# QuantumLiquids/PEPS

Hardware: AMD Instinct MI355X
Metric: configuration-amplitudes/sec (higher is better)
Workload: dtype f32

## Files before the change

### include/pepsgpu.h

```cpp
#ifndef PEPSGPU_H
#define PEPSGPU_H

#include <stddef.h>
#include <stdint.h>

#ifdef __cplusplus
extern "C" {
#endif

typedef struct pepsgpu_ctx pepsgpu_ctx;

enum {
  PEPSGPU_OK = 0,
  PEPSGPU_EINVAL = 1,
  PEPSGPU_EHIP = 2,
  PEPSGPU_ESTATE = 3,
  PEPSGPU_ERANGE = 4,
  PEPSGPU_EEMPTY = 5,
  PEPSGPU_ENOCONV = 6
};
enum { PEPSGPU_F32 = 0, PEPSGPU_F64 = 1, PEPSGPU_C128 = 3 };
enum { PEPSGPU_LEFT = 0, PEPSGPU_DOWN = 1, PEPSGPU_RIGHT = 2, PEPSGPU_UP = 3 };
enum { PEPSGPU_HORIZONTAL = 0, PEPSGPU_VERTICAL = 1 };
enum { PEPSGPU_SVD_COMPRESS = 0, PEPSGPU_VARIATION2SITE = 1, PEPSGPU_VARIATION1SITE = 2 };
// ... 203 lines not shown
int pepsgpu_comm_destroy(pepsgpu_ctx *ctx);
int pepsgpu_allreduce(pepsgpu_ctx *ctx, void *buf, long n, int dtype, int op, int on_device);
int pepsgpu_grad_allreduce(pepsgpu_ctx *ctx);
int pepsgpu_bcast_state(pepsgpu_ctx *ctx, int root);
int pepsgpu_grad_device_ptr(pepsgpu_ctx *ctx, void **so_dev, void **seo_dev, long *n_elems);

int pepsgpu_diag_tgemm(int dtype_in, int dtype_out, const int *desc_ints, int n_ints, const void *A, size_t a_elems,
                       const void *B, size_t b_elems, void *C, size_t c_elems, int nbatch, long wA, long wB, long wC);
int pepsgpu_diag_tgemm_desc(int types, const int *desc_ints, int n_ints, const long *desc_longs, int n_longs,
                            const double *desc_dbls, int n_dbls, const int32_t *pool, long pool_n, const float *scale_in,
                            const void *A, size_t a_elems, long a_offset, const void *B, size_t b_elems, long b_offset,
                            void *C, size_t c_elems, float *scale_out, double *norm_log, int32_t *norm_flag,
                            int32_t *route_out, unsigned long long *flops_out);
int pepsgpu_diag_tgemm_route(int types, const int *desc_ints, int n_ints, const long *desc_longs, int n_longs,
                             const double *desc_dbls, int n_dbls, long a_offset, long b_offset, int32_t *route_out);
int pepsgpu_diag_tgemm_chain3(const int *dims8, const int *site_strides4, long slot, int nslots, const int32_t *sel, int sel_inc,
                              const int32_t *live4, const int32_t *skip, int nbatch, const int *offs3, const float *mps1,
                              const float *bten, const float *site, const float *mps2, float *out, int32_t *flags_out,
                              int32_t *launched_out, int32_t *variant_out);
int pepsgpu_diag_dot4(int dtype, const void *a, const void *b, const int *dims4, int nbatch, const double *lsum, const int32_t *flag,
                      double *out);
int pepsgpu_diag_chol(int dtype_out, const double *G, int n, int nbatch, void *R_out);
int pepsgpu_diag_gram_cols(int dtype, const void *P, int K, int n, int nbatch, const int32_t *klive, double *G_out);
int pepsgpu_diag_gram_rows(const float *M, int n, int K, int nbatch, const int32_t *nrows, double *G_out);
int pepsgpu_diag_mgemm_dense(const float *R, const float *Tt, int m, int la, int a_dim, int u_dim, int k2_dim, int tt_u_inner, int nbatch,
                             const int32_t *m_live, const int32_t *a_live, const int32_t *k2_live, float *M_out);
int pepsgpu_diag_cg_stats(double *out16);
int pepsgpu_diag_lds_gram_chol(int which, const float *X, int n, int K, int nbatch, const int32_t *nlive, float *R_out, int32_t *mlive_out);
int pepsgpu_diag_chol_pivot(const float *X, int n, int K, int nbatch, const int32_t *nlive, int kcap, float *R_out, int32_t *mlive_out);
int pepsgpu_diag_rows_qr(const float *X, int k, int len, int nbatch, const int32_t *klive, float *V_out, int32_t *klive_out);
int pepsgpu_diag_suwa_todo(const double *weights, int n, int init, const uint32_t *words, int steps, int32_t *out_chain);
int pepsgpu_diag_tgemm_chain(const int *dims7, const int32_t *live3_per_entry, int nbatch, const float *R, const float *A,
                             const float *W, float *P_out, int32_t *flags_out);
int pepsgpu_diag_gram_chol(int dtype, const void *P, int K, int n, int nbatch, void *R_out, int32_t *mlive_out);
int pepsgpu_diag_gram_chol_wave(const float *P, int K, int n, int nbatch, const int32_t *klive, int inner,
                                const int32_t *inner_live, int max_pass, int form, float *R_out, int32_t *mlive_out);
int pepsgpu_diag_chol_adaptive(int dtype_out, const double *G, int n, int nbatch, void *R_out, int32_t *mlive_out);
int pepsgpu_diag_jacobi(int dtype, void *M, int m, int len, int nbatch, int k, void *Vt_out, void *S_out,
                        int force_global, int *sweeps_out);
int pepsgpu_diag_chol_solve_rows(int is_complex, const void *S, void *X, int nbatch, int r_max, int len, const int32_t *rows, int r,
                                 const int32_t *run_flag);
int pepsgpu_diag_gather_rows(int is_complex, const void *M, int nbatch, int m, int len, const int32_t *piv, int slots,
                             const int32_t *rows, const int32_t *run_flag, void *Q);
int pepsgpu_diag_sign_table(int is_complex, int rows, int cols, void *out);
int pepsgpu_diag_truncate_site(pepsgpu_ctx *ctx, const void *M, int nbatch, int m, int u, int k2, const int32_t *rows, int route,
                               void *V_out, int32_t *klive_out, int32_t *route_flag_out);
int pepsgpu_diag_trunc_rows(const float *M, int m, int len, int nbatch, const int32_t *rows, int k, int span, float *Vt_out,
                            int32_t *klive_out, int32_t *sweeps_out);
const char *pepsgpu_version(void);

#ifdef __cplusplus
}
#endif
#endif
```

### peps_amd/capi.py

```python
import ctypes as C
import os

import numpy as np

_HERE = os.path.dirname(os.path.abspath(__file__))
LIB_PATH = os.environ.get("PEPSGPU_LIB") or os.path.join(_HERE, "lib", "libpepsgpu.so")

F32, F64 = 0, 1
C128 = 3
LEFT, DOWN, RIGHT, UP = 0, 1, 2, 3
HORIZONTAL, VERTICAL = 0, 1
LEFTUP_TO_RIGHTDOWN, LEFTDOWN_TO_RIGHTUP = 0, 1
SVD_COMPRESS, VARIATION2SITE, VARIATION1SITE = 0, 1, 2

_ERR = {1: ValueError, 2: RuntimeError, 3: RuntimeError, 4: IndexError, 5: RuntimeError}

SYMBOLS = [
    "pepsgpu_ctx_create", "pepsgpu_set_truncate_params", "pepsgpu_ctx_destroy", "pepsgpu_last_error", "pepsgpu_state_upload",
    "pepsgpu_walkers_set_configs", "pepsgpu_walkers_get_configs", "pepsgpu_n_walkers",
    "pepsgpu_grow_bmps_step", "pepsgpu_grow_full_bmps", "pepsgpu_grow_bmps_for_row", "pepsgpu_grow_bmps_for_col",
    "pepsgpu_shift_bmps_window", "pepsgpu_delete_inner_bmps", "pepsgpu_bmps_park", "pepsgpu_bmps_unpark", "pepsgpu_generate_bmps_approach",
    "pepsgpu_sweep_slice_exchange", "pepsgpu_sweep_slice_exchange_tab", "pepsgpu_sweep_slice_fullspace", "pepsgpu_sweep_slice_tnn3", "pepsgpu_diag_tnn3_table", "pepsgpu_nn_exchange_slice", "pepsgpu_nn_exchange_slice_tab", "pepsgpu_onsite_slice", "pepsgpu_nnn_exchange_slice", "pepsgpu_diag_nnn_slice_calls", "pepsgpu_nnn_hop_slice_fermion", "pepsgpu_diag_nnn_hop_slice_calls", "pepsgpu_diag_fermion_hop_cand", "pepsgpu_nn_pair_slice_fermion", "pepsgpu_diag_pair_slice_calls", "pepsgpu_diag_pair_cand", "pepsgpu_nn_hop_slice_fermion", "pepsgpu_diag_hop_slice_calls", "pepsgpu_sweep_slice_sector", "pepsgpu_diag_sector_slice_calls", "pepsgpu_diag_sector_cand", "pepsgpu_link_exchange_slice", "pepsgpu_diag_link_slice_calls", "pepsgpu_diag_link_cand", "pepsgpu_walker_create", "pepsgpu_walker_clone", "pepsgpu_walker_destroy", "pepsgpu_walker_info", "pepsgpu_walker_set_mpo", "pepsgpu_walker_set_mpo_excited", "pepsgpu_walker_trace_slice", "pepsgpu_diag_walker_slice_calls", "pepsgpu_walker_set_mpo_excited_pair", "pepsgpu_walker_pair_trace_slice", "pepsgpu_diag_walker_pair_slice_calls", "pepsgpu_diag_walker_pair_cand", "pepsgpu_walker_evolve",
    "pepsgpu_walker_evolve_step", "pepsgpu_walker_contract_row", "pepsgpu_walker_init_bten", "pepsgpu_walker_grow_bten_step",
    "pepsgpu_walker_shift_bten_window", "pepsgpu_walker_trace_with_bten", "pepsgpu_walker_clear_bten", "pepsgpu_walker_get_bmps_tensor",
    "pepsgpu_bmps_stack_size", "pepsgpu_get_bmps_tensor", "pepsgpu_init_bten", "pepsgpu_grow_full_bten",
    "pepsgpu_grow_bten_step", "pepsgpu_shift_bten_window", "pepsgpu_truncate_bten", "pepsgpu_bten_stack_size",
    "pepsgpu_trace", "pepsgpu_replace_nn_trace", "pepsgpu_replace_one_trace", "pepsgpu_trace_scaling", "pepsgpu_punch_hole",
    "pepsgpu_init_bten2", "pepsgpu_grow_full_bten2", "pepsgpu_grow_bten2_step", "pepsgpu_shift_bten2_window",
    "pepsgpu_bten2_stack_size", "pepsgpu_replace_nnn_trace", "pepsgpu_replace_tnn_trace",
    "pepsgpu_bten2_select_set", "pepsgpu_cfg_override_slice", "pepsgpu_replace_plaquette_trace",
    "pepsgpu_replace_sqrt5_trace",
    "pepsgpu_grad_reset", "pepsgpu_grad_accumulate", "pepsgpu_grad_accumulate_states", "pepsgpu_grad_read", "pepsgpu_grad_device_ptr", "pepsgpu_grad_allreduce", "pepsgpu_bcast_state",
    "pepsgpu_comm_unique_id", "pepsgpu_comm_init", "pepsgpu_comm_size", "pepsgpu_comm_rank", "pepsgpu_comm_destroy",
    "pepsgpu_allreduce",
    "pepsgpu_sr_begin", "pepsgpu_sr_append", "pepsgpu_sr_count", "pepsgpu_sr_sum", "pepsgpu_sr_matvec", "pepsgpu_sr_matvec_c128",
    "pepsgpu_sr_cg_solve", "pepsgpu_sr_gram", "pepsgpu_sr_weighted_sum", "pepsgpu_sr_copy_samples",
    "pepsgpu_opt_begin", "pepsgpu_opt_end", "pepsgpu_opt_gradient_from_accumulators", "pepsgpu_opt_set_gradient",
    "pepsgpu_opt_get_gradient", "pepsgpu_opt_clip", "pepsgpu_opt_natural_gradient", "pepsgpu_opt_step", "pepsgpu_opt_scale_state",
    "pepsgpu_opt_read_state", "pepsgpu_fermion_decoration_set", "pepsgpu_minsr_direction", "pepsgpu_diag_eigh",
    "pepsgpu_vmc_snapshot_save", "pepsgpu_vmc_snapshot_read", "pepsgpu_vmc_snapshot_clear",
    "pepsgpu_guard_base_save", "pepsgpu_guard_base_restore", "pepsgpu_guard_base_clear", "pepsgpu_guard_preview",
    "pepsgpu_lbfgs_begin", "pepsgpu_lbfgs_end", "pepsgpu_lbfgs_reset", "pepsgpu_lbfgs_update", "pepsgpu_lbfgs_direction",
    "pepsgpu_lbfgs_trial", "pepsgpu_lbfgs_slope", "pepsgpu_lbfgs_commit", "pepsgpu_lbfgs_get_direction", "pepsgpu_lbfgs_get_pair",
    "pepsgpu_lbfgs_counters",
    "pepsgpu_update_local", "pepsgpu_erase_envs_after_update", "pepsgpu_evaluate_amplitude",
    "pepsgpu_walker_flags", "pepsgpu_sync", "pepsgpu_stats", "pepsgpu_profile_enable", "pepsgpu_profile_read",
    "pepsgpu_diag_tgemm", "pepsgpu_diag_tgemm_desc", "pepsgpu_diag_tgemm_route", "pepsgpu_diag_tgemm_chain", "pepsgpu_diag_tgemm_chain3", "pepsgpu_diag_chol", "pepsgpu_diag_chol_adaptive", "pepsgpu_diag_chol_pivot", "pepsgpu_diag_rows_qr", "pepsgpu_diag_suwa_todo", "pepsgpu_diag_dot4", "pepsgpu_diag_gram_chol", "pepsgpu_diag_gram_chol_wave", "pepsgpu_diag_gram_cols", "pepsgpu_diag_gram_rows", "pepsgpu_diag_mgemm_dense", "pepsgpu_diag_jacobi", "pepsgpu_diag_trunc_rows", "pepsgpu_version",
    "pepsgpu_diag_chol_solve_rows", "pepsgpu_diag_gather_rows", "pepsgpu_diag_sign_table", "pepsgpu_diag_truncate_site",
]


def load_library(path=LIB_PATH):
    if not os.path.exists(path):
        raise ImportError("libpepsgpu.so not built (%s): run `python -c 'import __graft_entry__ as g; g.build()'`" % path)
    lib = C.CDLL(path)
    vp, ip, dp = C.c_void_p, C.POINTER(C.c_int32), C.POINTER(C.c_double)
    lib.pepsgpu_ctx_create.argtypes = [C.POINTER(vp)] + [C.c_int] * 8 + [C.c_double, C.c_int, C.c_int]
    lib.pepsgpu_set_truncate_params.argtypes = [vp, C.c_int, C.c_int, C.c_double, C.c_int, C.c_double, C.c_int]
    lib.pepsgpu_ctx_destroy.argtypes = [vp]
    lib.pepsgpu_ctx_destroy.restype = None
    lib.pepsgpu_last_error.argtypes = [vp]
    lib.pepsgpu_last_error.restype = C.c_char_p
    lib.pepsgpu_version.restype = C.c_char_p
    lib.pepsgpu_state_upload.argtypes = [vp, vp, C.c_int]
    lib.pepsgpu_walkers_set_configs.argtypes = [vp, C.c_int, ip]
    lib.pepsgpu_walkers_get_configs.argtypes = [vp, ip]
    lib.pepsgpu_n_walkers.argtypes = [vp]
    for name in ("grow_bmps_step", "grow_full_bmps", "grow_bmps_for_row", "grow_bmps_for_col", "shift_bmps_window",
                 "delete_inner_bmps", "generate_bmps_approach", "bmps_stack_size", "bten_stack_size",
                 "grow_bten_step", "shift_bten_window"):
        getattr(lib, "pepsgpu_" + name).argtypes = [vp, C.c_int]
    lib.pepsgpu_bmps_park.argtypes = [vp, C.c_int, C.c_int]
    lib.pepsgpu_bmps_unpark.argtypes = [vp, C.c_int]
    lib.pepsgpu_get_bmps_tensor.argtypes = [vp, C.c_int, C.c_int, C.c_int, ip, dp, dp]
    lib.pepsgpu_init_bten.argtypes = [vp, C.c_int, C.c_int]
    lib.pepsgpu_truncate_bten.argtypes = [vp, C.c_int, C.c_int]
    lib.pepsgpu_grow_full_bten.argtypes = [vp, C.c_int, C.c_int, C.c_int, C.c_int]
    lib.pepsgpu_trace.argtypes = [vp, C.c_int, C.c_int, C.c_int, dp]
    lib.pepsgpu_replace_nn_trace.argtypes = [vp, C.c_int, C.c_int, C.c_int, C.c_int, ip, dp]
    lib.pepsgpu_replace_one_trace.argtypes = [vp, C.c_int, C.c_int, C.c_int, C.c_int, ip, dp]
    lib.pepsgpu_punch_hole.argtypes = [vp, C.c_int, C.c_int, C.c_int, dp]
# ... 965 lines not shown
    if sel.size < (nb - 1) * sel_inc + 1 or (sv.size - int(o3[2])) < slot * (int(sel.max()) + 1):
        raise ValueError("diag_tgemm_chain3: selector or site store too small")
    flags = np.full(nb, 7, dtype=np.int32)
    launched = np.zeros(1, dtype=np.int32)
    variant = np.zeros(3, dtype=np.int32)
    vpp = lambda a: a.ctypes.data_as(C.c_void_p)
    rc = lib().pepsgpu_diag_tgemm_chain3(_ip(d8), _ip(st), slot, (sv.size - int(offs[2])) // slot, _ip(sel), sel_inc,
                                         None if lv is None else _ip(lv), None if sk is None else _ip(sk), nb, _ip(o3),
                                         vpp(m1), vpp(bt), vpp(sv), vpp(m2), vpp(out), _ip(flags), _ip(launched), _ip(variant))
    if rc != 0:
        raise RuntimeError("diag_tgemm_chain3 failed: %s" % lib().pepsgpu_last_error(None).decode())
    return out, flags, int(launched[0]), tuple(int(v) for v in variant)


def diag_tgemm_chain(R, A, W, live):
    R = np.ascontiguousarray(R, dtype=np.float32); A = np.ascontiguousarray(A, dtype=np.float32)
    W = np.ascontiguousarray(W, dtype=np.float32)
    nb, m, l, a = R.shape
    _, _, p, a2 = A.shape
    l2, u = W.shape[3], W.shape[4]
    dims = np.array([m, l, a, p, a2, l2, u], dtype=np.int32)
    lv = np.ascontiguousarray(live, dtype=np.int32)
    P = np.zeros((nb, m, u, l2, a2), dtype=np.float32)
    fl = np.zeros(nb, dtype=np.int32)
    f = lib().pepsgpu_diag_tgemm_chain
    f.argtypes = [C.POINTER(C.c_int32), C.POINTER(C.c_int32), C.c_int, C.c_void_p, C.c_void_p, C.c_void_p, C.c_void_p, C.POINTER(C.c_int32)]
    rc = f(_ip(dims), _ip(lv), nb, R.ctypes.data_as(C.c_void_p), A.ctypes.data_as(C.c_void_p), W.ctypes.data_as(C.c_void_p),
           P.ctypes.data_as(C.c_void_p), _ip(fl))
    if rc != 0:
        raise RuntimeError("diag_tgemm_chain failed: %s" % lib().pepsgpu_last_error(None).decode())
    return P, fl


def diag_chol(dtype_out, G):
    G = np.ascontiguousarray(G, dtype=np.float64)
    nb, n, _ = G.shape
    R = np.zeros((nb, n, n), dtype=np.float32 if dtype_out == F32 else np.float64)
    rc = lib().pepsgpu_diag_chol(dtype_out, _dp(G), n, nb, R.ctypes.data_as(C.c_void_p))
    if rc != 0:
        raise RuntimeError("diag_chol failed: %s" % lib().pepsgpu_last_error(None).decode())
    return R


def diag_chol_adaptive(dtype_out, G):
    G = np.ascontiguousarray(G, dtype=np.float64)
    nb, n, _ = G.shape
    R = np.zeros((nb, n, n), dtype=np.float32 if dtype_out == F32 else np.float64)
    ml = np.zeros(nb, dtype=np.int32)
    rc = lib().pepsgpu_diag_chol_adaptive(dtype_out, _dp(G), n, nb, R.ctypes.data_as(C.c_void_p), _ip(ml))
    if rc != 0:
        raise RuntimeError("diag_chol_adaptive failed: %s" % lib().pepsgpu_last_error(None).decode())
    return R, ml


def diag_gram_chol(dtype, P):
    t = np.float32 if dtype == F32 else np.float64
    P = np.ascontiguousarray(P, dtype=t)
    nb, K, n = P.shape
    R = np.zeros((nb, n, n), dtype=t)
    ml = np.zeros(nb, dtype=np.int32)
    rc = lib().pepsgpu_diag_gram_chol(dtype, P.ctypes.data_as(C.c_void_p), K, n, nb, R.ctypes.data_as(C.c_void_p), _ip(ml))
    if rc != 0:
        raise RuntimeError("diag_gram_chol failed: %s" % lib().pepsgpu_last_error(None).decode())
    return R, ml


# ... 462 lines not shown
```

### peps_amd/csrc/capi.hip

```cpp
#include <cstring>
#include "../../include/pepsgpu.h"
#include "engine_impl.h"
#include "engine_nnn.h"
#include "engine_sr.h"
#include "engine_opt.h"
#include "engine_lbfgs.h"
#include "engine_guard.h"
#include "engine_var.h"
#include "engine_cplx.h"
#include "engine_walker.h"
#include "engine_sweep.h"
#include "comm.h"

using namespace pepsgpu;

namespace pepsgpu {
bool tgemm_use_mfma() {
  static int v = -1;
  if (v < 0) {
    const char *e = getenv("PEPSGPU_NO_MFMA");
    v = (e && e[0] == '1') ? 0 : 1;
  }
  return v == 1;
}
// ... 837 lines not shown
    PG_CHECK_HIP(hipMalloc(&dl, 3 * (size_t)nbatch * sizeof(int)));
    PG_CHECK_HIP(hipMalloc(&dflag, nbatch * sizeof(int)));
    PG_CHECK_HIP(hipMemcpy(dR, R, nR * nbatch * sizeof(float), hipMemcpyHostToDevice));
    PG_CHECK_HIP(hipMemcpy(dA, A, nA * nbatch * sizeof(float), hipMemcpyHostToDevice));
    PG_CHECK_HIP(hipMemcpy(dW, W, nW * nbatch * sizeof(float), hipMemcpyHostToDevice));
    PG_CHECK_HIP(hipMemset(dP, 0, nP * nbatch * sizeof(float)));
    std::vector<int> hl(3 * (size_t)nbatch);
    for (int b = 0; b < nbatch; ++b)
      for (int q = 0; q < 3; ++q) hl[(size_t)q * nbatch + b] = live[3 * b + q];
    PG_CHECK_HIP(hipMemcpy(dl, hl.data(), hl.size() * sizeof(int), hipMemcpyHostToDevice));
    const int *ml = dl, *al = dl + nbatch, *a2l = dl + 2 * nbatch;
    TGemmDesc gx, gp;
    gx.I[1] = m; gx.I[2] = l; gx.sAi[1] = l * a; gx.sAi[2] = a; gx.sCi[1] = l * p * a2; gx.sCi[2] = p * a2;
    gx.K[2] = a; gx.sAk[2] = 1; gx.sBk[2] = p * a2;
    gx.J[1] = p; gx.J[2] = a2; gx.sBj[1] = a2; gx.sBj[2] = 1; gx.sCj[1] = a2; gx.sCj[2] = 1;
    gx.wA = (long)nR; gx.wB = (long)nA; gx.wC = 0; gx.nbatch = nbatch;
    gx.dI[1].p = ml; gx.dK[2].p = al; gx.dJ[2].p = a2l;
    gp.I[1] = l2; gp.I[2] = u; gp.sAi[1] = u; gp.sAi[2] = 1; gp.sCi[1] = a2; gp.sCi[2] = l2 * a2;
    gp.K[1] = l; gp.K[2] = p; gp.sAk[1] = p * l2 * u; gp.sAk[2] = l2 * u;
    gp.J[1] = m; gp.J[2] = a2; gp.sCj[1] = u * l2 * a2; gp.sCj[2] = 1;
    gp.wA = (long)nW; gp.wC = (long)nP; gp.nbatch = nbatch;
    gp.dJ[1].p = ml; gp.dJ[2].p = a2l;
    TGemmChainMap mp;
    mp.mapK[1] = 2; mp.mapK[2] = 4;
    mp.mapJ[1] = 1; mp.mapJ[2] = 5;
    const char *f64_s = getenv("PEPSGPU_DIAG_CHAIN_F64");
    const char *tri_s = getenv("PEPSGPU_DIAG_TRI");
    PG_REQUIRE(tgemm_chain_launch(0, gx, gp, mp, dR, dA, dW, dP, dflag, 1, tri_s && atoi(tri_s) ? 1 : 0, f64_s && atoi(f64_s) ? 1 : 0,
                                  tri_s && atoi(tri_s) ? 1 : 0), 1, "chain launch refused");
    PG_CHECK_HIP(hipDeviceSynchronize());
    PG_CHECK_HIP(hipMemcpy(P_out, dP, nP * nbatch * sizeof(float), hipMemcpyDeviceToHost));
    PG_CHECK_HIP(hipMemcpy(flags_out, dflag, nbatch * sizeof(int), hipMemcpyDeviceToHost));
    (void)hipFree(dR); (void)hipFree(dA); (void)hipFree(dW); (void)hipFree(dP); (void)hipFree(dl); (void)hipFree(dflag);
  });
}

template <typename T>
static void diag_chol_t(const double *G, int n, int nbatch, void *Rout) {
  double *dG;
  T *dR;
  size_t ne = (size_t)n * n * nbatch;
  PG_CHECK_HIP(hipMalloc(&dG, ne * sizeof(double)));
  PG_CHECK_HIP(hipMalloc(&dR, ne * sizeof(T)));
  PG_CHECK_HIP(hipMemcpy(dG, G, ne * sizeof(double), hipMemcpyHostToDevice));
  launch_chol_upper<T>(0, nbatch, dG, (long)n * n, n, dR, (long)n * n, (int *)nullptr);
  PG_CHECK_HIP(hipDeviceSynchronize());
  PG_CHECK_HIP(hipMemcpy(Rout, dR, ne * sizeof(T), hipMemcpyDeviceToHost));
  (void)hipFree(dG); (void)hipFree(dR);
}
template <typename T>
static void diag_chol_adaptive_t(const double *G, int n, int nbatch, void *Rout, int32_t *mlive) {
  double *dG;
  T *dR;
  int *dml;
  size_t ne = (size_t)n * n * nbatch;
  PG_REQUIRE(n <= 256 * CH_LR_Q, 1, "n too large for the low-rank Cholesky");
  PG_CHECK_HIP(hipMalloc(&dG, ne * sizeof(double)));
  PG_CHECK_HIP(hipMalloc(&dR, ne * sizeof(T)));
  PG_CHECK_HIP(hipMalloc(&dml, nbatch * sizeof(int)));
  PG_CHECK_HIP(hipMemcpy(dG, G, ne * sizeof(double), hipMemcpyHostToDevice));
  PG_CHECK_HIP(hipMemset(dR, 0, ne * sizeof(T)));
  const size_t lsm = chol_lowrank_smem_bytes(n), smem = chol_smem_bytes(n);
  allow_dynamic_lds(reinterpret_cast<const void *>(&chol_lowrank_kernel<T>), lsm);
  allow_dynamic_lds(reinterpret_cast<const void *>(&chol_upper_kernel<T>), smem);
  hipLaunchKernelGGL(chol_lowrank_kernel<T>, dim3(nbatch), dim3(256), lsm, 0, (const double *)dG, (long)n * n, n, dR,
                     (long)n * n, dml);
// ... 505 lines not shown
```

### peps_amd/csrc/tgemm.h

```cpp
#pragma once
#include "common.h"
#include "cplx.h"

namespace pepsgpu {

struct TgDyn {
  const int *p = nullptr;
  int mul = 1;
  int mask = 0;
  int div = 1;
};

struct TGemmDesc {
  int I[3] = {1, 1, 1}, J[3] = {1, 1, 1}, K[3] = {1, 1, 1};
  int sAi[3] = {0, 0, 0}, sAk[3] = {0, 0, 0};
  int sBk[3] = {0, 0, 0}, sBj[3] = {0, 0, 0};
  int sCi[3] = {0, 0, 0}, sCj[3] = {0, 0, 0};
  long wA = 0, wB = 0, wC = 0;
  const int *selA = nullptr, *selB = nullptr;
  int selA_inc = 0, selB_inc = 0;
  long selA_mul = 0, selB_mul = 0;
  int bdivA = 1, bdivB = 1, bdivC = 1;
  int seldivA = 1, seldivB = 1;
  const int *dynI = nullptr, *dynK = nullptr;
  int dynI_mul = 1, dynK_mul = 1;
  TgDyn dI[3], dJ[3], dK[3];
  int Imask[3] = {0x7fffffff, 0x7fffffff, 0x7fffffff}, Jmask[3] = {0x7fffffff, 0x7fffffff, 0x7fffffff};
  int nbatch = 1;
  int accumulate = 0;
  int upper_only = 0;
  int conjA = 0, conjB = 0;
  const int *batch_flag = nullptr;
  unsigned long long *flopc = nullptr;
// ... 1177 lines not shown
      if (s == jsub) d2.J[s] = cn;
      if (s == mp3.chunkI) { d3.I[s] = cn; d3.Imask[s] = 0x7fffffff; }
    }
    {
      int st = 1;
      for (int s = 2; s >= 0; --s) { lds1[3 + s] = st; st *= d1.J[s]; }
      for (int s = 2; s >= 0; --s) { lds1[s] = st; st *= d1.I[s]; }
      st = 1;
      for (int s = 2; s >= 0; --s) { lds2[3 + s] = st; st *= d2.J[s]; }
      for (int s = 2; s >= 0; --s) { lds2[s] = st; st *= d2.I[s]; }
    }
#pragma unroll
    for (int s = 0; s < 3; ++s) {
      d1.sCi[s] = lds1[s]; d1.sCj[s] = lds1[3 + s];
      d2.sBk[s] = mp.mapK[s] >= 0 ? lds1[mp.mapK[s]] : 0;
      d2.sBj[s] = mp.mapJ[s] >= 0 ? lds1[mp.mapJ[s]] : 0;
      d2.sCi[s] = lds2[s]; d2.sCj[s] = lds2[3 + s];
      d3.sAi[s] = mp3.mapI[s] >= 0 ? lds2[mp3.mapI[s]] : 0;
      d3.sAk[s] = mp3.mapK[s] >= 0 ? lds2[mp3.mapK[s]] : 0;
    }
    if (c0) __syncthreads();
    tg_direct_body<AVEC1, BVEC1>(d1, A1g + baseA1 + (long)c0 * sA1, B1g + baseB1, s_mid1, d1.Itot(), J1, K2s1, offCi_s, 0, 4, in_scale);
    __syncthreads();
    tg_direct_body<AVEC2, false>(d2, A2g + baseA2, s_mid1, s_mid2, I2, d2.Jtot(), K2s2, offCi_s, 0, 4);
    __syncthreads();
    tg_direct_body<false, false>(d3, s_mid2, B3g + baseB3, C3 + (long)c0 * sC3, d3.Itot(), J3, K2s3, offCi_s, 0, 4);
  }
  if (n1 < x_static) {
    const long lo = (long)n1 * sC3, hi = (long)x_static * sC3;
    for (long e = lo + threadIdx.x; e < hi; e += 256) C3[e] = 0.f;
  }
}

inline int tgemm_chain_launch(hipStream_t s, const TGemmDesc &d1_in, const TGemmDesc &d2_in, const TGemmChainMap &mp,
                              const float *A1, const float *B1, const float *A2, float *C2, int *flag, int allow_chunks = 0, int dense = 0,
                              int f64acc = 0, int tri = 0);

inline int tgemm_chain3_launch(hipStream_t s, const TGemmDesc &d1_in, const TGemmDesc &d2_in, const TGemmDesc &d3_in, const TGemmChainMap &mp,
                               const TGemmChain3Map &mp3, const float *A1, const float *B1, const float *A2, const float *B3, float *C3, int *flag,
                               const int *skip = nullptr);

struct BTenChainDescs {
  TGemmDesc g1, g2, g3;
  TGemmChainMap mp;
  TGemmChain3Map mp3;
};
inline BTenChainDescs bten_chain_descs(int x, int p1, int cdim, int b1, int b2, int s1, int s2, int y, int st_c, int st_b, int st_1,
                                       int st_2, long wA1, long wB1, long wB3, const int *sel, int sel_inc, long slot, int nb,
                                       const int *vx, const int *vc, const int *vb, const int *vy) {
  BTenChainDescs c;
  TGemmDesc &g1 = c.g1, &g2 = c.g2, &g3 = c.g3;
  g1.I[1] = x; g1.I[2] = p1; g1.sAi[1] = p1 * cdim; g1.sAi[2] = cdim; g1.sCi[1] = p1 * b1 * b2; g1.sCi[2] = b1 * b2;
  g1.K[2] = cdim; g1.sAk[2] = 1; g1.sBk[2] = b1 * b2;
  g1.J[1] = b1; g1.J[2] = b2; g1.sBj[1] = b2; g1.sBj[2] = 1; g1.sCj[1] = b2; g1.sCj[2] = 1;
  g1.wA = wA1; g1.wB = wB1; g1.wC = (long)x * p1 * b1 * b2; g1.nbatch = nb;
  g1.dI[1].p = vx; g1.dK[2].p = vc; g1.dJ[2].p = vb;
  g2.I[1] = s1; g2.I[2] = s2; g2.sAi[1] = st_1; g2.sAi[2] = st_2; g2.sCi[1] = s2; g2.sCi[2] = 1;
  g2.K[1] = p1; g2.K[2] = b1; g2.sAk[1] = st_c; g2.sAk[2] = st_b; g2.sBk[1] = b1 * b2; g2.sBk[2] = b2;
  g2.J[1] = x; g2.J[2] = b2; g2.sBj[1] = p1 * b1 * b2; g2.sBj[2] = 1; g2.sCj[1] = s1 * s2; g2.sCj[2] = x * s1 * s2;
  g2.wB = g1.wC; g2.wC = (long)b2 * x * s1 * s2; g2.nbatch = nb;
  g2.dJ[1].p = vx; g2.dJ[2].p = vb;
  g2.selA = sel; g2.selA_mul = slot; g2.selA_inc = sel_inc; g2.seldivA = 1; g2.wA = 0;
  c.mp.mapK[1] = 2; c.mp.mapK[2] = 4;
  c.mp.mapJ[1] = 1; c.mp.mapJ[2] = 5;
  g3.I[1] = x; g3.I[2] = s2; g3.sCi[1] = s2 * y; g3.sCi[2] = y;
  g3.K[1] = b2; g3.K[2] = s1; g3.sBk[1] = s1 * y; g3.sBk[2] = y;
// ... 176 lines not shown
      break;
    case TG_ROUTE_SKINNY_128x32:
    case TG_ROUTE_SKINNY_32x128:
      if constexpr (std::is_same<TAcc, double>::value && !is_cplx<TA>::value && !is_cplx<TB>::value && !is_cplx<TC>::value) {
        if (r.kind == TG_ROUTE_SKINNY_128x32)
          hipLaunchKernelGGL((tgemm_skinny_f64_kernel<TA, TB, TC, 128, 32>), r.grid, dim3(256), 0, s, d, A, B, C);
        else
          hipLaunchKernelGGL((tgemm_skinny_f64_kernel<TA, TB, TC, 32, 128>), r.grid, dim3(256), 0, s, d, A, B, C);
      }
      break;
    case TG_ROUTE_TILED_MFMA:
      if constexpr (!is_cplx<TAcc>::value || std::is_same<TAcc, c128>::value)
        hipLaunchKernelGGL((tgemm_kernel<TA, TB, TC, TAcc, true>), r.grid, dim3(256), 0, s, d, A, B, C);
      break;
    default:
      hipLaunchKernelGGL((tgemm_kernel<TA, TB, TC, TAcc, false>), r.grid, dim3(256), 0, s, d, A, B, C);
      break;
  }
  PG_CHECK_HIP(hipGetLastError());
}

inline int tgemm_chain_launch(hipStream_t s, const TGemmDesc &d1_in, const TGemmDesc &d2_in, const TGemmChainMap &mp,
                              const float *A1, const float *B1, const float *A2, float *C2, int *flag, int allow_chunks, int dense, int f64acc,
                              int tri) {
  const int akf = (allow_chunks ? 1 : 0) | (tri ? 2 : 0);
  if (!tgemm_use_mfma() || d1_in.dynK || d2_in.dynK || d1_in.nbatch != d2_in.nbatch || d1_in.nbatch <= 0) return 0;
  if (d1_in.bdivA != 1 || d1_in.bdivB != 1 || d2_in.bdivA != 1 || d2_in.bdivC != 1) return 0;
  TGemmDesc d1 = d1_in, d2 = d2_in;
  if (d1.Itot() >= (1 << 22) || d1.Jtot() >= (1 << 22) || d2.Itot() >= (1 << 22) || d2.Jtot() >= (1 << 22)) return 0;
  d1.flopc = tg_flop_counter; d1.bytec = tg_byte_counter;
  d1.flop_stride = d1.nbatch >= 256 ? 64 : 1;
  d1.thin = d2.thin = tgemm_thin() & TG_THIN_TILES;
  d1.stage_span = d2.stage_span = 0;
  constexpr bool no_vec = false;
  const bool avec1 = !no_vec && tg_vec_a(d1, A1), bvec1 = !no_vec && tg_vec_b(d1, B1), avec2 = !no_vec && tg_vec_a(d2, A2);
  const dim3 g(d1.nbatch), blk(256);
  int ldsf = (dense && allow_chunks) ? 8192 : TG_CHAIN_LDS_FLOATS;
  if (f64acc && ldsf > 8192) ldsf = 8192;
#define PG_CHAIN(a1, b1, a2)                                                                                                   \
  do {                                                                                                                         \
    if (f64acc && ldsf >= 8192) hipLaunchKernelGGL((tgemm_chain_kernel<a1, b1, a2, 8192, 4, true>), g, blk, 0, s, d1, d2, mp, A1, B1, A2, C2, flag, 0, akf); \
    else if (f64acc) hipLaunchKernelGGL((tgemm_chain_kernel<a1, b1, a2, TG_CHAIN_LDS_FLOATS, 4, true>), g, blk, 0, s, d1, d2, mp, A1, B1, A2, C2, flag, 0, akf); \
    else if (ldsf == 8192 && tri) hipLaunchKernelGGL((tgemm_chain_kernel<a1, b1, a2, 8192, 4, false, true>), g, blk, 0, s, d1, d2, mp, A1, B1, A2, C2, flag, 0, akf); \
    else if (ldsf == 8192) hipLaunchKernelGGL((tgemm_chain_kernel<a1, b1, a2, 8192, 4>), g, blk, 0, s, d1, d2, mp, A1, B1, A2, C2, flag, 0, akf); \
    else hipLaunchKernelGGL((tgemm_chain_kernel<a1, b1, a2, TG_CHAIN_LDS_FLOATS, 6>), g, blk, 0, s, d1, d2, mp, A1, B1, A2, C2, flag, 0, akf); \
  } while (0)
  if (avec1 && bvec1 && avec2) PG_CHAIN(true, true, true);
  else if (avec1 && bvec1) PG_CHAIN(true, true, false);
  else if (avec1 && avec2) PG_CHAIN(true, false, true);
  else if (avec1) PG_CHAIN(true, false, false);
  else if (bvec1 && avec2) PG_CHAIN(false, true, true);
  else if (bvec1) PG_CHAIN(false, true, false);
  else if (avec2) PG_CHAIN(false, false, true);
  else PG_CHAIN(false, false, false);
#undef PG_CHAIN
  PG_CHECK_HIP(hipGetLastError());
  int jsub = -1;
  for (int q = 0; q < 3; ++q) {
    if (mp.mapJ[q] == 1) jsub = (jsub < 0 && !(d2.dJ[q].p && d2.dJ[q].mask)) ? q : 3;
    if (mp.mapK[q] == 1) jsub = 3;
  }
  const long whole = (long)d1.Itot() * d1.Jtot(), per = (long)d1.I[2] * d1.Jtot();
  const bool chunkable = allow_chunks && d1.I[0] == 1 && !d1.dynI && !d2.dynI && jsub >= 0 && jsub <= 2 &&
                         !(d1.dI[1].p && d1.dI[1].mask) && per <= ldsf;
  return (whole <= ldsf || chunkable) ? 2 : 1;
}
// ... 17 lines not shown
    if (mp.mapJ[q] == 1) jsub = (jsub < 0 && !(d2.dJ[q].p && d2.dJ[q].mask)) ? q : 3;
    if (mp.mapK[q] == 1) jsub = 3;
  }
  if (jsub < 0 || jsub > 2 || mp3.chunkI < 0 || mp3.chunkI > 2 || d1.I[0] != 1 || (d1.dI[1].p && d1.dI[1].mask)) return 0;
  if (mp3.mapI[mp3.chunkI] != 3 + jsub) return 0;
  for (int q = 0; q < mp3.chunkI; ++q) if (d3.I[q] != 1) return 0;
  const long per1 = (long)d1.I[2] * d1.Jtot(), per2 = (long)d2.Itot() * d2.Jtot() / (d2.J[jsub] > 0 ? d2.J[jsub] : 1);
  if (per1 > ldsf || per2 > ldsf) return 0;
  d1.flopc = tg_flop_counter; d1.bytec = tg_byte_counter;
  d1.flop_stride = d1.nbatch >= 256 ? 64 : 1;
  d1.thin = d2.thin = d3.thin = tgemm_thin() & TG_THIN_TILES;
  d1.stage_span = d2.stage_span = d3.stage_span = 0;
  constexpr bool no_vec = false;
  const bool avec1 = !no_vec && tg_vec_a(d1, A1), bvec1 = !no_vec && tg_vec_b(d1, B1), avec2 = !no_vec && tg_vec_a(d2, A2);
  const dim3 g(d1.nbatch), blk(256);
#define PG_CHAIN3(a1, b1, a2)                                                                                                               \
  do {                                                                                                                                      \
    hipLaunchKernelGGL((tgemm_chain3_kernel<a1, b1, a2, 4096, 4>), g, blk, 0, s, d1, d2, d3, mp, mp3, A1, B1, A2, B3, C3, flag, skip);   \
  } while (0)
  if (avec1 && bvec1 && avec2) PG_CHAIN3(true, true, true);
  else if (avec1 && bvec1) PG_CHAIN3(true, true, false);
  else if (avec1 && avec2) PG_CHAIN3(true, false, true);
  else if (avec1) PG_CHAIN3(true, false, false);
  else if (bvec1 && avec2) PG_CHAIN3(false, true, true);
  else if (bvec1) PG_CHAIN3(false, true, false);
  else if (avec2) PG_CHAIN3(false, false, true);
  else PG_CHAIN3(false, false, false);
#undef PG_CHAIN3
  PG_CHECK_HIP(hipGetLastError());
  return 2;
}

}
```

Before: 149,100.

## Add specialized MFMA chain kernel for bond-dimension-8 two-GEMM contractions

Adds a dedicated fused two-GEMM chain kernel for the case where the inner bond dimensions are 8. It uses 32x32x2 f32 MFMA tiles, stages the intermediate in padded LDS, and chunks over x when the intermediate does not fit. The generic chain dispatcher routes matching descriptors to it by default, with an environment switch to disable it, plus diagnostic entry points and counters. The goal is to replace the generic templated chain kernel's indexing and tile overhead on this common shape. The cost is a new code path whose strict acceptance checks and masking logic must exactly reproduce the generic results.

```diff
diff --git a/include/pepsgpu.h b/include/pepsgpu.h
--- a/include/pepsgpu.h
+++ b/include/pepsgpu.h
@@ -259,6 +259,11 @@
 int pepsgpu_diag_suwa_todo(const double *weights, int n, int init, const uint32_t *words, int steps, int32_t *out_chain);
 int pepsgpu_diag_tgemm_chain(const int *dims7, const int32_t *live3_per_entry, int nbatch, const float *R, const float *A,
                              const float *W, float *P_out, int32_t *flags_out);
+int pepsgpu_diag_tgemm_chain_pair(int backward, const int *dims8, const int *site_strides4, long slot, int nslots, const int32_t *sel,
+                                  const int32_t *live3_per_entry, int nbatch, int opts, const float *scale_in, const float *op1,
+                                  const float *op2, const float *site, float *out, int32_t *flags_out, int32_t *info_out);
+long pepsgpu_diag_chain_d8_launches(void);
+int pepsgpu_diag_chain_d8_stats(unsigned long long *out2);
 int pepsgpu_diag_gram_chol(int dtype, const void *P, int K, int n, int nbatch, void *R_out, int32_t *mlive_out);
 int pepsgpu_diag_gram_chol_wave(const float *P, int K, int n, int nbatch, const int32_t *klive, int inner,
                                 const int32_t *inner_live, int max_pass, int form, float *R_out, int32_t *mlive_out);
diff --git a/peps_amd/capi.py b/peps_amd/capi.py
--- a/peps_amd/capi.py
+++ b/peps_amd/capi.py
@@ -47,6 +47,7 @@
     "pepsgpu_walker_flags", "pepsgpu_sync", "pepsgpu_stats", "pepsgpu_profile_enable", "pepsgpu_profile_read",
     "pepsgpu_diag_tgemm", "pepsgpu_diag_tgemm_desc", "pepsgpu_diag_tgemm_route", "pepsgpu_diag_tgemm_chain", "pepsgpu_diag_tgemm_chain3", "pepsgpu_diag_chol", "pepsgpu_diag_chol_adaptive", "pepsgpu_diag_chol_pivot", "pepsgpu_diag_rows_qr", "pepsgpu_diag_suwa_todo", "pepsgpu_diag_dot4", "pepsgpu_diag_gram_chol", "pepsgpu_diag_gram_chol_wave", "pepsgpu_diag_gram_cols", "pepsgpu_diag_gram_rows", "pepsgpu_diag_mgemm_dense", "pepsgpu_diag_jacobi", "pepsgpu_diag_trunc_rows", "pepsgpu_version",
     "pepsgpu_diag_chol_solve_rows", "pepsgpu_diag_gather_rows", "pepsgpu_diag_sign_table", "pepsgpu_diag_truncate_site",
+    "pepsgpu_diag_tgemm_chain_pair", "pepsgpu_diag_chain_d8_launches", "pepsgpu_diag_chain_d8_stats",
 ]
 
 
@@ -1078,6 +1079,57 @@
     return P, fl
 
 
+def diag_tgemm_chain_pair(backward, dims, site_strides, site, slot, sel, op1, op2, live, out_init, d8=True, tsw=False,
+                          zero_fill=False, f64=False, scale_in=None):
+    d8v = np.ascontiguousarray(dims, dtype=np.int32)
+    st = np.ascontiguousarray(site_strides, dtype=np.int32)
+    sel = np.ascontiguousarray(sel, dtype=np.int32)
+    f32 = lambda a: np.ascontiguousarray(a, dtype=np.float32).ravel()
+    o1, o2, sv = f32(op1), f32(op2), f32(site)
+    out = np.ascontiguousarray(out_init, dtype=np.float32).copy()
+    nb = int(out.shape[0])
+    lv = np.ascontiguousarray(live, dtype=np.int32)
+    m, a, a2, k2, l, p, l2, u = (int(v) for v in d8v)
+    n1, n2, no = ((a * p * a2, l2 * a2 * k2, l * a * u * k2) if backward else (m * l * a, a * p * a2, m * u * l2 * a2))
+    if o1.size != n1 * nb or o2.size != n2 * nb or out.size != no * nb or lv.size != 3 * nb or sel.size != nb or d8v.size != 8:
+        raise ValueError("diag_tgemm_chain_pair: operand sizes do not match dims")
+    if sv.size % slot or int(sel.min()) < 0 or (int(sel.max()) + 1) * slot > sv.size:
+        raise ValueError("diag_tgemm_chain_pair: selector or site store too small")
+    reach = sum((e - 1) * int(s) for e, s in zip((l, p, l2, u), st))
+    if reach >= slot or int(st.min()) < 0:
+        raise ValueError("diag_tgemm_chain_pair: site strides reach beyond a slot")
+    sc = None if scale_in is None else np.ascontiguousarray(scale_in, dtype=np.float32)
+    flags = np.full(nb, 7, dtype=np.int32)
+    info = np.zeros(2, dtype=np.int32)
+    vpp = lambda x: x.ctypes.data_as(C.c_void_p)
+    f = lib().pepsgpu_diag_tgemm_chain_pair
+    f.argtypes = [C.c_int, C.POINTER(C.c_int32), C.POINTER(C.c_int32), C.c_long, C.c_int, C.POINTER(C.c_int32), C.POINTER(C.c_int32),
+                  C.c_int, C.c_int, C.c_void_p, C.c_void_p, C.c_void_p, C.c_void_p, C.c_void_p, C.POINTER(C.c_int32),
+                  C.POINTER(C.c_int32)]
+    opts = (1 if d8 else 0) | (2 if tsw else 0) | (4 if zero_fill else 0) | (8 if f64 else 0)
+    rc = f(1 if backward else 0, _ip(d8v), _ip(st), slot, sv.size // slot, _ip(sel), _ip(lv), nb, opts,
+           None if sc is None else vpp(sc), vpp(o1), vpp(o2), vpp(sv), vpp(out), _ip(flags), _ip(info))
+    if rc != 0:
+        raise RuntimeError("diag_tgemm_chain_pair failed: %s" % lib().pepsgpu_last_error(None).decode())
+    return out, flags, int(info[0]), bool(info[1])
+
+
+def diag_chain_d8_launches():
+    f = lib().pepsgpu_diag_chain_d8_launches
+    f.argtypes = []
+    f.restype = C.c_long
+    return int(f())
+
+
+def diag_chain_d8_stats():
+    out = (C.c_ulonglong * 2)()
+    f = lib().pepsgpu_diag_chain_d8_stats
+    f.argtypes = [C.POINTER(C.c_ulonglong)]
+    if f(out) != 0:
+        raise RuntimeError("diag_chain_d8_stats failed: %s" % lib().pepsgpu_last_error(None).decode())
+    return int(out[0]), int(out[1])
+
+
 def diag_chol(dtype_out, G):
     G = np.ascontiguousarray(G, dtype=np.float64)
     nb, n, _ = G.shape
diff --git a/peps_amd/csrc/capi.hip b/peps_amd/csrc/capi.hip
--- a/peps_amd/csrc/capi.hip
+++ b/peps_amd/csrc/capi.hip
@@ -893,6 +893,73 @@
     PG_CHECK_HIP(hipMemcpy(P_out, dP, nP * nbatch * sizeof(float), hipMemcpyDeviceToHost));
     PG_CHECK_HIP(hipMemcpy(flags_out, dflag, nbatch * sizeof(int), hipMemcpyDeviceToHost));
     (void)hipFree(dR); (void)hipFree(dA); (void)hipFree(dW); (void)hipFree(dP); (void)hipFree(dl); (void)hipFree(dflag);
+  });
+}
+
+extern "C" int pepsgpu_diag_tgemm_chain_pair(int backward, const int *dims8, const int *site_strides4, long slot, int nslots,
+                                             const int32_t *sel, const int32_t *live3, int nbatch, int opts, const float *scale_in,
+                                             const float *op1, const float *op2, const float *site, float *out, int32_t *flags_out,
+                                             int32_t *info_out) {
+  return guarded(nullptr, [&]() {
+    PG_REQUIRE(nbatch > 0 && nslots > 0 && slot > 0 && dims8 && site_strides4 && sel && live3 && op1 && op2 && site && out, 1, "bad arguments");
+    SiteDims d;
+    d.m = dims8[0]; d.a = dims8[1]; d.a2 = dims8[2]; d.k2 = dims8[3]; d.l = dims8[4]; d.p = dims8[5]; d.l2 = dims8[6]; d.u = dims8[7];
+    d.ll = 0; d.lp = 1; d.lr = 2; d.lu = 3;
+    for (int q = 0; q < 4; ++q) d.st[q] = site_strides4[q];
+    d.la = d.l * d.a; d.uk = d.u * d.k2;
+    for (int b = 0; b < nbatch; ++b) PG_REQUIRE(sel[b] >= 0 && sel[b] < nslots, 1, "selector beyond the site store");
+    const long n1 = backward ? (long)d.a * d.p * d.a2 : (long)d.m * d.l * d.a;
+    const long n2 = backward ? (long)d.l2 * d.a2 * d.k2 : (long)d.a * d.p * d.a2;
+    const long no = backward ? (long)d.l * d.a * d.u * d.k2 : (long)d.m * d.u * d.l2 * d.a2;
+    DevBufs mb;
+    const float *d1p = mb.alloc<float>(n1 * nbatch, op1), *d2p = mb.alloc<float>(n2 * nbatch, op2);
+    const float *dsite = mb.alloc<float>((size_t)slot * nslots, site);
+    float *dout = mb.alloc<float>(no * nbatch, out);
+    const int *dsel = mb.alloc<int>(nbatch, sel);
+    const float *dscale = scale_in ? mb.alloc<float>(nbatch, scale_in) : nullptr;
+    int *dflag = mb.alloc<int>(nbatch, flags_out);
+    std::vector<int> hl(3 * (size_t)nbatch);
+    for (int b = 0; b < nbatch; ++b)
+      for (int q = 0; q < 3; ++q) hl[(size_t)q * nbatch + b] = live3[3 * b + q];
+    const int *dl = mb.alloc<int>(hl.size(), hl.data());
+    const int *v0 = dl, *v1 = dl + nbatch, *v2 = dl + 2 * (size_t)nbatch;
+    TGemmDesc g1, g2;
+    if (backward) {
+      g1 = desc_z1(d, n1, n2, 0, nbatch, v0, v1, v2);
+      g1.scale_in = dscale;
+      g2 = desc_tt(d, (opts & 2) != 0, 0, no, nbatch, v0, v2, (opts & 4) != 0);
+    } else {
+      g1 = desc_x(d, n1, n2, 0, nbatch, v0, 1, v1, v2);
+      g2 = desc_p(d, 0, no, nbatch, v0, 1, v2);
+    }
+    g2.selA = dsel; g2.selA_mul = slot; g2.selA_inc = 1; g2.seldivA = 1; g2.wA = 0;
+    TGemmChainMap mp;
+    mp.mapK[1] = 2; mp.mapK[2] = 4;
+    mp.mapJ[1] = 1; mp.mapJ[2] = 5;
+    const long before = tg_chain_d8_count.load();
+    tg_chain_d8_force = (opts & 1) ? 1 : 0;
+    int rc = 0;
+    try {
+      rc = tgemm_chain_launch(0, g1, g2, mp, d1p, d2p, dsite, dout, dflag, 1, 0, (opts & 8) ? 1 : 0);
+    } catch (...) { tg_chain_d8_force = -1; throw; }
+    tg_chain_d8_force = -1;
+    PG_REQUIRE(rc != 0, 1, "chain launch refused");
+    PG_CHECK_HIP(hipDeviceSynchronize());
+    info_out[0] = rc;
+    info_out[1] = tg_chain_d8_count.load() != before ? 1 : 0;
+    PG_CHECK_HIP(hipMemcpy(out, dout, no * nbatch * sizeof(float), hipMemcpyDeviceToHost));
+    PG_CHECK_HIP(hipMemcpy(flags_out, dflag, nbatch * sizeof(int), hipMemcpyDeviceToHost));
+  });
+}
+
+extern "C" long pepsgpu_diag_chain_d8_launches(void) { return tg_chain_d8_count.load(); }
+extern "C" int pepsgpu_diag_chain_d8_stats(unsigned long long *out2) {
+  return guarded(nullptr, [&]() {
+    out2[0] = out2[1] = 0;
+    if (const unsigned long long *p = tgemm_chain_d8_stats()) {
+      PG_CHECK_HIP(hipDeviceSynchronize());
+      PG_CHECK_HIP(hipMemcpy(out2, p, 2 * sizeof(unsigned long long), hipMemcpyDeviceToHost));
+    }
   });
 }
 
diff --git a/peps_amd/csrc/tgemm.h b/peps_amd/csrc/tgemm.h
--- a/peps_amd/csrc/tgemm.h
+++ b/peps_amd/csrc/tgemm.h
@@ -1,4 +1,5 @@
 #pragma once
+#include <atomic>
 #include "common.h"
 #include "cplx.h"
 
@@ -1242,6 +1243,28 @@
   }
 }
 
+inline bool tgemm_chain_d8_enabled() {
+  static const bool v = !(getenv("PEPSGPU_CHAIN_D8") && atoi(getenv("PEPSGPU_CHAIN_D8")) == 0);
+  return v;
+}
+inline thread_local int tg_chain_d8_force = -1;
+inline std::atomic<long> tg_chain_d8_count{0};
+inline unsigned long long *tgemm_chain_d8_stats() {
+  static unsigned long long *p = []() -> unsigned long long * {
+    const char *e = getenv("PEPSGPU_CHAIN_D8_STATS");
+    if (!e || !atoi(e)) return nullptr;
+    unsigned long long *q = nullptr;
+    if (hipMalloc(&q, 2 * sizeof(unsigned long long)) != hipSuccess) return nullptr;
+    (void)hipMemset(q, 0, 2 * sizeof(unsigned long long));
+    return q;
+  }();
+  return p;
+}
+inline bool tgemm_chain_d8_accepts(const TGemmDesc &d1, const TGemmDesc &d2, const TGemmChainMap &mp, const float *A1, int allow_chunks,
+                                   int dense, int f64acc);
+inline int tgemm_chain_d8_launch(hipStream_t s, const TGemmDesc &d1, const TGemmDesc &d2, const float *A1, const float *B1, const float *A2,
+                                 float *C2, int *flag);
+
 inline int tgemm_chain_launch(hipStream_t s, const TGemmDesc &d1_in, const TGemmDesc &d2_in, const TGemmChainMap &mp,
                               const float *A1, const float *B1, const float *A2, float *C2, int *flag, int allow_chunks = 0, int dense = 0,
                               int f64acc = 0, int tri = 0);
@@ -1484,6 +1507,9 @@
   d1.flop_stride = d1.nbatch >= 256 ? 64 : 1;
   d1.thin = d2.thin = tgemm_thin() & TG_THIN_TILES;
   d1.stage_span = d2.stage_span = 0;
+  if ((tg_chain_d8_force >= 0 ? tg_chain_d8_force != 0 : tgemm_chain_d8_enabled()) &&
+      tgemm_chain_d8_accepts(d1, d2, mp, A1, allow_chunks, dense, f64acc))
+    return tgemm_chain_d8_launch(s, d1, d2, A1, B1, A2, C2, flag);
   constexpr bool no_vec = false;
   const bool avec1 = !no_vec && tg_vec_a(d1, A1), bvec1 = !no_vec && tg_vec_b(d1, B1), avec2 = !no_vec && tg_vec_a(d2, A2);
   const dim3 g(d1.nbatch), blk(256);
@@ -1567,3 +1593,5 @@
 }
 
 }
+
+#include "tgemm_d8.h"
diff --git a/peps_amd/csrc/tgemm_d8.h b/peps_amd/csrc/tgemm_d8.h
--- /dev/null
+++ b/peps_amd/csrc/tgemm_d8.h
@@ -0,0 +1,250 @@
+#pragma once
+#include "tgemm.h"
+
+namespace pepsgpu {
+
+constexpr int TG_D8_COLS = TG_CHAIN_LDS_FLOATS / 64;
+constexpr int TG_D8_PITCH = TG_D8_COLS + 1;
+
+struct TgChainD8Args {
+  const float *A1, *B1, *W;
+  float *C2;
+  int *flag;
+  const int *xl, *kl, *yl, *sel;
+  const float *scale_in;
+  unsigned long long *flopc, *bytec;
+  unsigned long long *stats;
+  long wA1, wB1, wW, wC2, sel_mul;
+  int sel_inc, xmul, X, Ks, Ys;
+  int sA_i1, sA_i2;
+  int sB_k, sB_j1, sB_j2;
+  int sW_i1, sW_i2, sW_k1, sW_k2;
+  int sC_i1, sC_i2, sC_j1, sC_j2;
+  float alpha1, alpha2;
+  int flop_stride;
+};
+
+__global__ __launch_bounds__(256, 6) void tgemm_chain_d8_kernel(const TgChainD8Args a) {
+  __shared__ float s_mid[64 * TG_D8_PITCH];
+  __shared__ int s_ocj[TG_D8_COLS];
+  const int b = blockIdx.x;
+  const int tid = threadIdx.x, lane = tid & 63, half = lane >> 5, l31 = lane & 31;
+  const int wave = __builtin_amdgcn_readfirstlane(tid >> 6);
+
+  int x, K, y, wsel;
+  float in_scale;
+  {
+    typedef const __attribute__((address_space(4))) int *cint_p;
+    typedef const __attribute__((address_space(4))) float *cfloat_p;
+    const int *const nz = &tg_neutral_word;
+    const int *px = a.xl ? a.xl + b : nz, *pk = a.kl ? a.kl + b : nz, *py = a.yl ? a.yl + b : nz;
+    const int *ps = a.sel ? a.sel + (long)b * a.sel_inc : nz;
+    const float *pc = a.scale_in ? a.scale_in + b : reinterpret_cast<const float *>(nz);
+    asm volatile("" ::"s"(px), "s"(pk), "s"(py), "s"(ps), "s"(pc));
+    const int vx = *(cint_p)px, vk = *(cint_p)pk, vy = *(cint_p)py, vs = *(cint_p)ps;
+    const float vc = *(cfloat_p)pc;
+    asm volatile("" ::"s"(vx), "s"(vk), "s"(vy), "s"(vs), "s"(vc));
+    x = a.xl ? max(0, min(a.X, vx * a.xmul)) : a.X;
+    K = a.kl ? max(0, min(a.Ks, vk)) : a.Ks;
+    y = a.yl ? max(0, min(a.Ys, vy)) : a.Ys;
+    wsel = a.sel ? vs : 0;
+    in_scale = a.scale_in ? vc : 1.f;
+  }
+  int chunk = x;
+  if (64 * x * y > TG_CHAIN_LDS_FLOATS) {
+    if (y > TG_D8_COLS) {
+      if (tid == 0) a.flag[b] = -1;
+      return;
+    }
+    chunk = 1;
+    while ((chunk + 1) * y <= TG_D8_COLS) ++chunk;
+  }
+  if (tid == 0) a.flag[b] = 0;
+  if (x <= 0 || y <= 0) return;
+  if (a.flopc && tid == 0 && (b & (a.flop_stride - 1)) == 0) {
+    const unsigned long long I1 = 8ull * x, J1 = 8ull * y, J2 = (unsigned long long)x * y;
+    atomicAdd(a.flopc, 2ull * a.flop_stride * (I1 * J1 * K + 64ull * J2 * 64ull));
+    if (a.bytec) atomicAdd(a.bytec, 4ull * a.flop_stride * (I1 * K + K * J1 + 64ull * 64ull + 64ull * J2));
+  }
+  if (a.stats && tid == 0) {
+    atomicAdd(a.stats, 1ull);
+    if (chunk < x) atomicAdd(a.stats + 1, 1ull);
+  }
+  const float *A1 = a.A1 + (long)b * a.wA1;
+  const float *B1 = a.B1 + (long)b * a.wB1;
+  const float *W = a.W + (long)b * a.wW + (long)wsel * a.sel_mul;
+  float *C2 = a.C2 + (long)b * a.wC2;
+  const float alpha1 = a.alpha1 * in_scale, alpha2 = a.alpha2;
+
+  {
+    const int sh = y <= 32 ? 5 : 7;
+    const int yv = tid & ((1 << sh) - 1);
+    for (int xl = tid >> sh; xl < chunk; xl += 256 >> sh)
+      if (yv < y) s_ocj[xl * y + yv] = xl * a.sC_j1 + yv * a.sC_j2;
+  }
+
+  const int rowA = (l31 >> 3) * a.sA_i1 + (l31 & 7) * a.sA_i2;
+  const int colB = (l31 >> 2) * a.sB_j1;
+  const unsigned sBk = (unsigned)a.sB_k;
+  const int ti2 = wave & 1;
+  unsigned wq[4];
+  {
+    const int rowW = (ti2 * 4 + (l31 >> 3)) * a.sW_i1 + (l31 & 7) * a.sW_i2;
+#pragma unroll
+    for (int q = 0; q < 4; ++q) wq[q] = 4u * (unsigned)(rowW + (4 * half + q) * a.sW_k2);
+  }
+  const int rowC = ti2 * 4 * a.sC_i1 + 4 * half * a.sC_i2;
+  const int nr8 = (K + 7) >> 3;
+  const int ntj1 = (y + 3) >> 2;
+
+  for (int c0 = 0; c0 < x; c0 += chunk) {
+    const int cn = min(chunk, x - c0);
+    if (c0) __syncthreads();
+    {
+      const float *Ac = A1 + (long)c0 * a.sA_i1;
+      const int nti = (cn + 3) >> 2;
+      int ti = 0, tj = wave;
+      while (tj >= ntj1) { tj -= ntj1; ++ti; }
+      while (ti < nti) {
+        const unsigned oab = (ti * 4 + (l31 >> 3) < cn) ? 4u * (unsigned)(rowA + ti * 4 * a.sA_i1) : 0u;
+        const int yv = tj * 4 + (l31 & 3);
+        const bool jv = yv < y;
+        const unsigned obb = 4u * (unsigned)(colB + (jv ? yv : 0) * a.sB_j2);
+        tg_f32x16 acc;
+#pragma unroll
+        for (int r = 0; r < 16; ++r) acc[r] = 0.f;
+        auto load_round = [&](const int r, float (&av)[4], float (&bv)[4]) {
+          const int kq = 8 * r + 4 * half;
+          const float4 v = tg_ldf4(Ac, oab + 4u * (unsigned)min(kq, a.Ks - 4));
+          av[0] = v.x; av[1] = v.y; av[2] = v.z; av[3] = v.w;
+#pragma unroll
+          for (int q = 0; q < 4; ++q) bv[q] = tg_ldf(B1, obb + 4u * __umul24((unsigned)min(kq + q, K - 1), sBk));
+        };
+        auto mfma_round = [&](const int r, float (&av)[4], float (&bv)[4]) {
+          const int left = K - 8 * r;
+          if (left < 8) {
+            const int kq = 8 * r + 4 * half;
+#pragma unroll
+            for (int q = 0; q < 4; ++q) {
+              const bool ok = kq + q < K;
+              av[q] = ok ? av[q] : 0.f;
+              bv[q] = ok ? bv[q] : 0.f;
+            }
+          }
+          acc = __builtin_amdgcn_mfma_f32_32x32x2f32(av[0], bv[0], acc, 0, 0, 0);
+          if (left > 1) acc = __builtin_amdgcn_mfma_f32_32x32x2f32(av[1], bv[1], acc, 0, 0, 0);
+          if (left > 2) acc = __builtin_amdgcn_mfma_f32_32x32x2f32(av[2], bv[2], acc, 0, 0, 0);
+          if (left > 3) acc = __builtin_amdgcn_mfma_f32_32x32x2f32(av[3], bv[3], acc, 0, 0, 0);
+        };
+        for (int r = 0; r < nr8; r += 2) {
+          float a0[4], b0[4], a1[4], b1[4];
+          const bool two = r + 1 < nr8;
+          load_round(r, a0, b0);
+          if (two) load_round(r + 1, a1, b1);
+          mfma_round(r, a0, b0);
+          if (two) mfma_round(r + 1, a1, b1);
+        }
+        if (jv) {
+          float *o = s_mid + ((4 * half * 8 + (l31 >> 2)) * TG_D8_PITCH + ti * 4 * y + yv);
+#pragma unroll
+          for (int g = 0; g < 4; ++g) {
+            if (ti * 4 + g < cn) {
+#pragma unroll
+              for (int e = 0; e < 4; ++e) o[e * 8 * TG_D8_PITCH] = acc[4 * g + e] * alpha1;
+            }
+            o += y;
+          }
+        }
+        tj += 4;
+        while (tj >= ntj1) { tj -= ntj1; ++ti; }
+      }
+    }
+    float w[8][4];
+    {
+      unsigned wo[4] = {wq[0], wq[1], wq[2], wq[3]};
+      asm volatile("" : "+v"(wo[0]), "+v"(wo[1]), "+v"(wo[2]), "+v"(wo[3]));
+#pragma unroll
+      for (int k1 = 0; k1 < 8; ++k1) {
+        const float *Wk = W + (long)k1 * a.sW_k1;
+#pragma unroll
+        for (int q = 0; q < 4; ++q) w[k1][q] = tg_ldf(Wk, wo[q]);
+      }
+    }
+    __syncthreads();
+    {
+      const int Jt = cn * y;
+      float *Cc = C2 + (long)c0 * a.sC_j1;
+      for (int j0 = (wave >> 1) * 32; j0 < Jt; j0 += 64) {
+        const int j = j0 + l31;
+        const float *bp = s_mid + (4 * half * TG_D8_PITCH + j);
+        tg_f32x16 acc;
+#pragma unroll
+        for (int r = 0; r < 16; ++r) acc[r] = 0.f;
+#pragma unroll
+        for (int k1 = 0; k1 < 8; ++k1)
+#pragma unroll
+          for (int q = 0; q < 4; ++q) acc = __builtin_amdgcn_mfma_f32_32x32x2f32(w[k1][q], bp[(k1 * 8 + q) * TG_D8_PITCH], acc, 0, 0, 0);
+        if (j < Jt) {
+          const unsigned oc = 4u * (unsigned)(s_ocj[j] + rowC);
+#pragma unroll
+          for (int g = 0; g < 4; ++g)
+#pragma unroll
+            for (int e = 0; e < 4; ++e)
+              *reinterpret_cast<float *>(reinterpret_cast<char *>(Cc + (long)(g * a.sC_i1 + e * a.sC_i2)) + oc) = acc[4 * g + e] * alpha2;
+        }
+      }
+    }
+  }
+}
+
+inline bool tgemm_chain_d8_accepts(const TGemmDesc &d1, const TGemmDesc &d2, const TGemmChainMap &mp, const float *A1, int allow_chunks,
+                                   int dense, int f64acc) {
+  if (!allow_chunks || dense || f64acc) return false;
+  if (mp.mapK[0] != -1 || mp.mapK[1] != 2 || mp.mapK[2] != 4 || mp.mapJ[0] != -1 || mp.mapJ[1] != 1 || mp.mapJ[2] != 5) return false;
+  if (d1.I[0] != 1 || d1.K[0] != 1 || d1.K[1] != 1 || d1.J[0] != 1 || d2.I[0] != 1 || d2.K[0] != 1 || d2.J[0] != 1) return false;
+  if (d1.I[2] != 8 || d1.J[1] != 8 || d2.I[1] != 8 || d2.I[2] != 8 || d2.K[1] != 8 || d2.K[2] != 8) return false;
+  if (d2.J[1] != d1.I[1] || d2.J[2] != d1.J[2] || d1.I[1] < 1 || d1.J[2] < 1 || d1.K[2] < 4) return false;
+  if (!tg_vec_a(d1, A1)) return false;
+  auto unset = [](const TgDyn &t) { return t.p == nullptr; };
+  auto plain = [](const TgDyn &t) { return t.p == nullptr || (t.mask == 0 && t.div == 1); };
+  auto same = [](const TgDyn &s, const TgDyn &t) { return s.p == t.p && (s.p == nullptr || (s.mul == t.mul && s.mask == t.mask && s.div == t.div)); };
+  if (!unset(d1.dI[0]) || !unset(d1.dI[2]) || !unset(d1.dJ[0]) || !unset(d1.dJ[1]) || !unset(d1.dK[0]) || !unset(d1.dK[1])) return false;
+  for (int s = 0; s < 3; ++s)
+    if (!unset(d2.dI[s]) || !unset(d2.dK[s])) return false;
+  if (!unset(d2.dJ[0]) || !plain(d1.dI[1]) || !plain(d1.dK[2]) || !plain(d1.dJ[2])) return false;
+  if (!same(d1.dI[1], d2.dJ[1]) || !same(d1.dJ[2], d2.dJ[2])) return false;
+  if ((d1.dK[2].p && d1.dK[2].mul != 1) || (d1.dJ[2].p && d1.dJ[2].mul != 1) || (d1.dI[1].p && d1.dI[1].mul < 1)) return false;
+  if (d1.dynI || d2.dynI || d1.selA || d1.selB || d2.selB || d2.accumulate || d2.seldivA != 1) return false;
+  const int st[] = {d1.sAi[1], d1.sAi[2], d1.sBk[2], d1.sBj[1], d1.sBj[2], d2.sAi[1], d2.sAi[2], d2.sAk[1], d2.sAk[2],
+                    d2.sCi[1], d2.sCi[2], d2.sCj[1], d2.sCj[2]};
+  for (int v : st)
+    if (v < 0 || v >= (1 << 24)) return false;
+  const long spanA = (long)d1.I[1] * d1.sAi[1] + 8l * d1.sAi[2] + d1.K[2];
+  const long spanB = (long)d1.K[2] * d1.sBk[2] + 8l * d1.sBj[1] + (long)d1.J[2] * d1.sBj[2];
+  const long spanW = 8l * (d2.sAi[1] + d2.sAi[2] + d2.sAk[1] + d2.sAk[2]);
+  const long spanC = 8l * (d2.sCi[1] + d2.sCi[2]) + (long)d2.J[1] * d2.sCj[1] + (long)d2.J[2] * d2.sCj[2];
+  return spanA < (1l << 29) && spanB < (1l << 29) && spanW < (1l << 29) && spanC < (1l << 29);
+}
+
+inline int tgemm_chain_d8_launch(hipStream_t s, const TGemmDesc &d1, const TGemmDesc &d2, const float *A1, const float *B1, const float *A2,
+                                 float *C2, int *flag) {
+  TgChainD8Args a;
+  a.A1 = A1; a.B1 = B1; a.W = A2; a.C2 = C2; a.flag = flag;
+  a.xl = d1.dI[1].p; a.kl = d1.dK[2].p; a.yl = d1.dJ[2].p; a.sel = d2.selA; a.scale_in = d1.scale_in;
+  a.flopc = d1.flopc; a.bytec = d1.bytec;
+  a.stats = tgemm_chain_d8_stats();
+  a.wA1 = d1.wA; a.wB1 = d1.wB; a.wW = d2.wA; a.wC2 = d2.wC; a.sel_mul = d2.selA_mul;
+  a.sel_inc = d2.selA_inc; a.xmul = d1.dI[1].mul; a.X = d1.I[1]; a.Ks = d1.K[2]; a.Ys = d1.J[2];
+  a.sA_i1 = d1.sAi[1]; a.sA_i2 = d1.sAi[2];
+  a.sB_k = d1.sBk[2]; a.sB_j1 = d1.sBj[1]; a.sB_j2 = d1.sBj[2];
+  a.sW_i1 = d2.sAi[1]; a.sW_i2 = d2.sAi[2]; a.sW_k1 = d2.sAk[1]; a.sW_k2 = d2.sAk[2];
+  a.sC_i1 = d2.sCi[1]; a.sC_i2 = d2.sCi[2]; a.sC_j1 = d2.sCj[1]; a.sC_j2 = d2.sCj[2];
+  a.alpha1 = (float)d1.alpha; a.alpha2 = (float)d2.alpha;
+  a.flop_stride = d1.flop_stride;
+  hipLaunchKernelGGL(tgemm_chain_d8_kernel, dim3(d1.nbatch), dim3(256), 0, s, a);
+  PG_CHECK_HIP(hipGetLastError());
+  tg_chain_d8_count.fetch_add(1, std::memory_order_relaxed);
+  return d1.J[2] <= TG_D8_COLS ? 2 : 1;
+}
+
+}
```

After: 156,800, median of 6. 5.1% higher.
